# haidog-yaqub/EzAudio

Hardware: AMD Instinct MI355X
Metric: denoising steps/sec (EzAudio-XL, 10 s latent, CFG on) (higher is better)
Workload: dtype bf16

## Files before the change

ezaudio_amd/csrc/attn.hip:

```cpp
#include "common.h"

namespace {

typedef __attribute__((ext_vector_type(4))) short s16x4;

__device__ __forceinline__ float pair_max(float x) {
    const auto r = __builtin_amdgcn_permlane32_swap(__float_as_uint(x), __float_as_uint(x), false, false);
    return fmaxf(__uint_as_float(r[0]), __uint_as_float(r[1]));
}
__device__ __forceinline__ float pair_sum(float x) {
    const auto r = __builtin_amdgcn_permlane32_swap(__float_as_uint(x), __float_as_uint(x), false, false);
    return __uint_as_float(r[0]) + __uint_as_float(r[1]);
}

template <int DH>
struct HeadGeom;
template <>
struct HeadGeom<64> { static constexpr int DQK = 64, DV = 64; };
template <>
struct HeadGeom<72> { static constexpr int DQK = 80, DV = 96; };

template <int DH, int NKH, bool ZQ = false, int QT = 64>
__global__ __launch_bounds__(128 * NKH) void k_attn(AttnArgs a) {
    static_assert(QT == 64 || (QT == 32 && NKH == 4), "32-query tiles: the 8-wave fused-projection form only");
    constexpr int NQS = QT / 32;
    constexpr int NT = 128 * NKH;
    constexpr int TK = 32 * NKH;
    constexpr int DQK = HeadGeom<DH>::DQK;
    constexpr int DV = HeadGeom<DH>::DV;
    constexpr int NKS = DQK / 16;
    constexpr int NDT = DV / 32;
    constexpr int KSTR = DQK * 2 + 16;
    constexpr int VSTR = 192;
    static_assert(DV * 2 <= VSTR, "V row");
    constexpr int KBYTES = TK * KSTR, VBYTES = TK * VSTR;
    constexpr int BUF = KBYTES + VBYTES;
    constexpr int KCH = TK * DQK * 2 / 16;
    constexpr int VCPR = DV / 8;
    constexpr int VCH = TK * VCPR;
    constexpr int KPT = (KCH + NT - 1) / NT, VPT = (VCH + NT - 1) / NT;
    static_assert(KPT <= 3 && VPT <= 3, "staging registers");
    constexpr int DN = DV >= 96 ? 96 : 64;
    constexpr int DW = DQK;
    constexpr int DS = DQK;
    constexpr int NRS = QT == 64 ? 3 : 4;
    constexpr int PSTAGE = (QT + DN) * 128, PRING = 2 * NRS * PSTAGE;
    constexpr int PRED = 4 * 64 * DS * 4, PQS = QT * DQK * 2;
    constexpr int SMEM = NKH == 4 ? (2 * BUF > PRED + PQS ? (2 * BUF > PRING ? 2 * BUF : PRING) : (PRED + PQS > PRING ? PRED + PQS : PRING)) : 2 * BUF;
    constexpr int ZX = ZQ ? QT * 8 + 2 * DQK * 4 : 0;
    __shared__ __attribute__((aligned(16))) char smem[SMEM + ZX];

    int Lq_ = a.Lq;
    asm("" : "+s"(Lq_) : "s"(a.q), "s"(a.k), "s"(a.v), "s"(a.kmask), "s"(a.out), "s"(a.ldo), "s"(a.B), "s"(a.H), "s"(a.Lk), "s"(a.Lqp), "s"(a.Lkp), "s"(a.xu), "s"(a.ldu),
        "s"(a.xw), "s"(a.ldw), "s"(a.xw_rows), "s"(a.xK), "s"(a.xcd_map), "s"(a.nq), "s"(a.ppx), "s"(a.mnq), "s"(a.mH), "s"(a.q_raw), "s"(a.ts), "s"(a.xk2), "s"(a.zstat_in),
        "s"(a.zs_stride), "s"(a.zparts), "s"(a.klen));
    const int tid = threadIdx.x;
    const int lane = tid & 63;
    const int wave = tid >> 6;
    const int qs = QT == 64 ? (wave & 1) : 0, kh = QT == 64 ? (wave >> 1) : (wave & 3);
    const bool active = QT == 64 || __builtin_amdgcn_readfirstlane(wave) < 4;
    const int r32 = lane & 31, hi = lane >> 5;
    int qt, h, b;
    if (a.xcd_map) {
        const int xcd = blockIdx.x & 7, sl = blockIdx.x >> 3;
        const int sq = ez_div(sl, a.mnq);
        const int pair = xcd * a.ppx + sq;
        qt = sl - sq * a.nq;
        if (pair >= a.B * a.H) return;
        b = ez_div(pair, a.mH); h = pair - b * a.H;
    } else {
        qt = blockIdx.x; h = blockIdx.y; b = blockIdx.z;
    }
    const int q0 = qt * QT + qs * 32;
    const long bh = (long)b * a.H + h;
    int Lk = a.Lk;
    if constexpr (!ZQ) {
        if (a.klen) {
            Lk = __builtin_amdgcn_readfirstlane(a.klen[b]);
            if (qt * QT >= Lk) {
                for (int i = tid; i < QT * (DH / 4); i += NT) {
                    const int r = i / (DH / 4), g = i - r * (DH / 4);
                    if (qt * QT + r < a.Lq)
                        *reinterpret_cast<uint2*>(a.out + ((long)b * a.Lq + qt * QT + r) * a.ldo + h * DH + 4 * g) = make_uint2(0u, 0u);
                }
                return;
            }
        }
    }
    unsigned long long* ts = (a.ts && tid < 64) ? a.ts + 8 * (long)blockIdx.x : nullptr;
    if (ts && lane == 0) { ts[0] = __builtin_readcyclecounter(); ts[6] = ez_stamp_start(); }

    const bf16_t* Q = a.q + (bh * a.Lqp + q0 + r32) * DQK + 8 * hi;
    const char* Kg = reinterpret_cast<const char*>(a.k + bh * a.Lkp * DQK);
    const bf16_t* Vg = a.v + bh * DV * (long)a.Lkp;
    const uint8_t* km = a.kmask ? a.kmask + (long)b * a.Lk : nullptr;

    bf16x8 qf[NKS];
    if (NKH == 4 && a.xu) {
        if constexpr (NKH == 4) {
            constexpr int FN = DN / 32;
            constexpr int NPART = QT == 64 ? 4 : 8;
            const int rowb = b * a.Lq;
            float2* zrow_l = reinterpret_cast<float2*>(smem + SMEM);
            float* zgc_l = reinterpret_cast<float*>(smem + SMEM + QT * 8);
            ZStatRegs zst;
            float4 zgc_reg = make_float4(0.f, 0.f, 0.f, 0.f);
            const int wave_u = __builtin_amdgcn_readfirstlane(wave);
            const char* gA = reinterpret_cast<const char*>(a.xu);
            const char* gW = reinterpret_cast<const char*>(a.xw);
            const int nt = a.xK / 64;
            auto z_request = [&]() {
                if constexpr (ZQ) {
                    if (tid < 4 * QT) {
                        int qr = qt * QT + (tid >> 2);
                        qr = qr < a.Lq ? qr : a.Lq - 1;
                        z_row_stats_load(a.zstat_in + (rowb + qr), a.zs_stride, a.zparts, tid & 3, zst);
                    }
                    if (tid < 2 * (DH / 4)) {
                        const int which = tid >= DH / 4, t4 = tid - which * (DH / 4);
                        zgc_reg = *reinterpret_cast<const float4*>((which ? a.zC : a.zG) + h * DH + 4 * t4);
                    }
                }
            };
            f32x16 acc[FN];
#pragma unroll
            for (int j = 0; j < FN; ++j)
#pragma unroll
                for (int r = 0; r < 16; ++r) acc[j][r] = 0.f;
            if constexpr (QT == 32) {
                constexpr int NCH = (32 + DW) * 8, NW1 = (NCH - NT) / 64;
                static_assert(NCH > NT && NCH <= 2 * NT && (NCH - NT) % 64 == 0, "two passes, whole waves");
                uint32_t off0, off1;
                {
                    const int row = tid >> 3, c = tid & 7;
                    if (row < 32) {
                        int grow = rowb + qt * 32 + row;
                        grow = grow < rowb + a.Lq - 1 ? grow : rowb + a.Lq - 1;
                        off0 = (uint32_t)(grow * a.ldu + ((c ^ ((row >> 1) & 7)) << 3)) * 2u;
                    } else {
                        const int r2 = row - 32;
                        int gr = h * DH + r2;
                        gr = gr < a.xw_rows - 1 ? gr : a.xw_rows - 1;
                        off0 = (uint32_t)(gr * a.ldw + ((c ^ ((r2 >> 1) & 7)) << 3)) * 2u;
                    }
                    const int r2 = (tid >> 3) + 32;
                    int gr = h * DH + r2;
                    gr = gr < a.xw_rows - 1 ? gr : a.xw_rows - 1;
                    off1 = (uint32_t)(gr * a.ldw + ((c ^ ((r2 >> 1) & 7)) << 3)) * 2u;
                }
                const char* g0 = wave_u < 4 ? gA : gW;
                const bool two = wave_u < NW1;
                auto stage2 = [&](int sidx) {
                    char* dst = smem + (sidx % NRS) * 2 * PSTAGE + wave_u * 1024;
#pragma unroll
                    for (int sub = 0; sub < 2; ++sub) {
                        const long ko = (long)(2 * sidx + sub) * 128;
                        __builtin_amdgcn_global_load_lds((const __attribute__((address_space(1))) void*)(g0 + ko + off0),
                                                         (__attribute__((address_space(3))) void*)(dst + sub * PSTAGE), 16, 0, 0);
                        if (two)
                            __builtin_amdgcn_global_load_lds((const __attribute__((address_space(1))) void*)(gW + ko + off1),
                                                             (__attribute__((address_space(3))) void*)(dst + sub * PSTAGE + NT * 16), 16, 0, 0);
                    }
                };
                const int ns = nt >> 1;
                stage2(0);
                z_request();
                if (ns > 1) stage2(1);
                if (ns > 2) stage2(2);
                const int sub = wave_u >> 2, kq = wave_u & 3;
                const uint32_t fo = r32 * 128 + (((2 * kq + hi) ^ ((r32 >> 1) & 7)) << 4);
                for (int sidx = 0; sidx < ns; ++sidx) {
                    const int younger = ns - 1 - sidx < NRS - 2 ? ns - 1 - sidx : NRS - 2;
                    if (two) {
                        if (younger >= 2) asm volatile("s_waitcnt vmcnt(8)" ::: "memory");
                        else if (younger == 1) asm volatile("s_waitcnt vmcnt(4)" ::: "memory");
                        else asm volatile("s_waitcnt vmcnt(0)" ::: "memory");
                    } else {
                        if (younger >= 2) asm volatile("s_waitcnt vmcnt(4)" ::: "memory");
                        else if (younger == 1) asm volatile("s_waitcnt vmcnt(2)" ::: "memory");
                        else asm volatile("s_waitcnt vmcnt(0)" ::: "memory");
                    }
                    __builtin_amdgcn_s_barrier();
                    if (sidx + NRS - 1 < ns) stage2(sidx + NRS - 1);
                    const char* cT = smem + (sidx % NRS) * 2 * PSTAGE + sub * PSTAGE;
                    const bf16x8 af = *reinterpret_cast<const bf16x8*>(cT + fo);
#pragma unroll
                    for (int j = 0; j < FN; ++j) {
                        const bf16x8 bfr = *reinterpret_cast<const bf16x8*>(cT + 32 * 128 + fo + j * 4096);
                        acc[j] = __builtin_amdgcn_mfma_f32_32x32x16_bf16(bfr, af, acc[j], 0, 0, 0);
                    }
#pragma unroll
                    for (int j = 0; j < FN; ++j) asm volatile("" : "+a"(acc[j]));
                }
            } else {
            const int mh = wave & 1, kq = wave >> 1;
            uint32_t aoff[1], boff[(DW * 8 + NT - 1) / NT];
            stage_offsets<64, NT>(aoff, a.ldu, rowb + qt * 64, rowb + a.Lq - 1, tid);
            stage_offsets<DW, NT>(boff, a.ldw, h * DH, a.xw_rows - 1, tid);
            auto stage = [&](int t) {
                char* dst = smem + (t % 3) * PSTAGE + wave_u * 1024;
                stage_tile<64, NT>(gA + (long)t * 128, aoff, dst, tid);
                stage_tile<DW, NT>(gW + (long)t * 128, boff, dst + 64 * 128, tid);
            };
            const bool two = (DW * 8 > NT) && (wave_u * 64 + NT < DW * 8);
            stage(0);
            if (nt > 1) stage(1);
            z_request();
            const uint32_t fo = r32 * 128 + (((2 * kq + hi) ^ ((r32 >> 1) & 7)) << 4);
            if (a.xk2 && (nt & 1) == 0) {
                const int ns = nt >> 1;
                auto stage2 = [&](int sidx) {
                    char* dst = smem + (sidx % 3) * 2 * PSTAGE + wave_u * 1024;
#pragma unroll
                    for (int sub = 0; sub < 2; ++sub) {
                        stage_tile<64, NT>(gA + (long)(2 * sidx + sub) * 128, aoff, dst + sub * PSTAGE, tid);
                        stage_tile<DW, NT>(gW + (long)(2 * sidx + sub) * 128, boff, dst + sub * PSTAGE + 64 * 128, tid);
                    }
                };
                if (ns > 1) stage2(1);
                for (int sidx = 0; sidx < ns; ++sidx) {
                    if (sidx + 1 < ns) {
                        if (two) asm volatile("s_waitcnt vmcnt(6)" ::: "memory"); else asm volatile("s_waitcnt vmcnt(4)" ::: "memory");
                    } else {
                        asm volatile("s_waitcnt vmcnt(0)" ::: "memory");
                    }
                    __builtin_amdgcn_s_barrier();
                    if (sidx + 2 < ns) stage2(sidx + 2);
#pragma unroll
                    for (int sub = 0; sub < 2; ++sub) {
                        const char* cT = smem + (sidx % 3) * 2 * PSTAGE + sub * PSTAGE;
                        const bf16x8 af = *reinterpret_cast<const bf16x8*>(cT + fo + mh * 4096);
#pragma unroll
                        for (int j = 0; j < FN; ++j) {
                            const bf16x8 bfr = *reinterpret_cast<const bf16x8*>(cT + 64 * 128 + fo + j * 4096);
                            acc[j] = __builtin_amdgcn_mfma_f32_32x32x16_bf16(bfr, af, acc[j], 0, 0, 0);
                        }
                    }
#pragma unroll
                    for (int j = 0; j < FN; ++j) asm volatile("" : "+a"(acc[j]));
                }
            } else
            for (int t = 0; t < nt; ++t) {
                if (t + 1 < nt) {
                    if (two) asm volatile("s_waitcnt vmcnt(3)" ::: "memory"); else asm volatile("s_waitcnt vmcnt(2)" ::: "memory");
                } else {
                    asm volatile("s_waitcnt vmcnt(0)" ::: "memory");
                }
                __builtin_amdgcn_s_barrier();
                if (t + 2 < nt) stage(t + 2);
                const char* cT = smem + (t % 3) * PSTAGE;
                const bf16x8 af = *reinterpret_cast<const bf16x8*>(cT + fo + mh * 4096);
#pragma unroll
                for (int j = 0; j < FN; ++j) {
                    const bf16x8 bfr = *reinterpret_cast<const bf16x8*>(cT + 64 * 128 + fo + j * 4096);
                    acc[j] = __builtin_amdgcn_mfma_f32_32x32x16_bf16(bfr, af, acc[j], 0, 0, 0);
                }
#pragma unroll
                for (int j = 0; j < FN; ++j) asm volatile("" : "+a"(acc[j]));
            }
            }
#pragma unroll
            for (int j = 0; j < FN; ++j) asm volatile("s_nop 7\n\ts_nop 7\n\ts_nop 3" : "+a"(acc[j]));
            if constexpr (ZQ) {
                if (tid < 4 * QT) {
                    const float2 mr = z_row_stats_finish(zst, a.zparts, tid & 3, a.zD, a.zeps);
                    if ((tid & 3) == 0) zrow_l[tid >> 2] = mr;
                }
                if (tid < 2 * (DH / 4)) {
                    const int which = tid >= DH / 4, t4 = tid - which * (DH / 4);
                    *reinterpret_cast<float4*>(zgc_l + which * DQK + 4 * t4) = zgc_reg;
                }
            }
            __syncthreads();
            float* red = reinterpret_cast<float*>(smem);
            {
                const int pw = QT == 64 ? (wave >> 1) : wave, prow = QT == 64 ? 32 * (wave & 1) + r32 : r32;
#pragma unroll
                for (int j = 0; j < FN; ++j)
#pragma unroll
                    for (int g = 0; g < 4; ++g) {
                        const int col = 32 * j + 8 * g + 4 * hi;
                        if (col < DS)
                            *reinterpret_cast<float4*>(red + ((pw * QT + prow) * DS + col)) =
                                make_float4(acc[j][4 * g], acc[j][4 * g + 1], acc[j][4 * g + 2], acc[j][4 * g + 3]);
                    }
            }
            __syncthreads();
            if (QT == 64 || tid < 8 * QT) {
                constexpr int CP = DH / 8;
                bf16_t* qs_l = reinterpret_cast<bf16_t*>(smem + PRED);
                const int row = tid >> 3, part = tid & 7;
                float v[CP];
                float s1 = 0.f;
                const float2 zmr = ZQ ? zrow_l[row] : make_float2(0.f, 1.f);
                const float zmu = zmr.x, zr = zmr.y;
#pragma unroll
                for (int e = 0; e < CP; ++e) {
                    const int col = part * CP + e;
                    if constexpr (QT == 64) {
                        v[e] = red[(0 * 64 + row) * DS + col] + red[(1 * 64 + row) * DS + col] + red[(2 * 64 + row) * DS + col] +
                               red[(3 * 64 + row) * DS + col];
                    } else {
                        float t = red[row * DS + col];
#pragma unroll
                        for (int w = 1; w < NPART; ++w) t += red[(w * QT + row) * DS + col];
                        v[e] = t;
                    }
                    if constexpr (ZQ) v[e] = fmaf(zr, v[e], fmaf(-zr * zmu, zgc_l[col], zgc_l[DQK + col]));
                    s1 += v[e];
                }
                s1 = oct_sum(s1);
                const float mean = s1 * (1.f / DH);
                float s2 = 0.f;
#pragma unroll
                for (int e = 0; e < CP; ++e) { const float d = v[e] - mean; s2 += d * d; }
                s2 = oct_sum(s2);
                const float rstd = rsqrtf(s2 * (1.f / DH) + 1e-5f);
#pragma unroll
                for (int e = 0; e < CP; ++e) {
                    const int col = part * CP + e;
                    qs_l[row * DQK + col] = f2bf((v[e] - mean) * rstd * a.qn_w[col] + a.qn_b[col]);
                }
                if (DQK > DH && part == 0)
                    for (int col = DH; col < DQK; ++col) qs_l[row * DQK + col] = 0;
            }
            __syncthreads();
            {
                const bf16_t* qs_l = reinterpret_cast<const bf16_t*>(smem + PRED);
#pragma unroll
                for (int ks = 0; ks < NKS; ++ks) qf[ks] = *reinterpret_cast<const bf16x8*>(qs_l + (32 * qs + r32) * DQK + 16 * ks + 8 * hi);
            }
            __syncthreads();
        }
    } else if (a.q_raw) {
        int qr = q0 + r32;
        if (qr >= a.Lq) qr = a.Lq - 1;
        const float* src = a.q_raw + ((long)b * a.Lq + qr) * a.ld_qraw + h * DH + 8 * hi;
        float v[NKS][8];
        float s = 0.f;
#pragma unroll
        for (int ks = 0; ks < NKS; ++ks) {
            const bool ok = 16 * ks + 8 * hi < DH;
            const float4 lo = ok ? *reinterpret_cast<const float4*>(src + 16 * ks) : make_float4(0.f, 0.f, 0.f, 0.f);
            const float4 hh = ok ? *reinterpret_cast<const float4*>(src + 16 * ks + 4) : make_float4(0.f, 0.f, 0.f, 0.f);
            v[ks][0] = lo.x; v[ks][1] = lo.y; v[ks][2] = lo.z; v[ks][3] = lo.w;
            v[ks][4] = hh.x; v[ks][5] = hh.y; v[ks][6] = hh.z; v[ks][7] = hh.w;
#pragma unroll
            for (int e = 0; e < 8; ++e) s += v[ks][e];
        }
        s += __shfl_xor(s, 32, 64);
        const float mean = s * (1.f / DH);
        float q2 = 0.f;
#pragma unroll
        for (int ks = 0; ks < NKS; ++ks)
            if (16 * ks + 8 * hi < DH) {
#pragma unroll
                for (int e = 0; e < 8; ++e) { const float d = v[ks][e] - mean; q2 += d * d; }
            }
        q2 += __shfl_xor(q2, 32, 64);
        const float rstd = rsqrtf(q2 * (1.f / DH) + 1e-5f);
#pragma unroll
        for (int ks = 0; ks < NKS; ++ks) {
            const int d0 = 16 * ks + 8 * hi;
            const bool ok = d0 < DH;
            const int dw = ok ? d0 : 0;
            union { bf16x8 v; uint32_t u[4]; } pk;
#pragma unroll
            for (int e = 0; e < 4; ++e) {
                const float y0 = ok ? (v[ks][2 * e] - mean) * rstd * a.qn_w[dw + 2 * e] + a.qn_b[dw + 2 * e] : 0.f;
                const float y1 = ok ? (v[ks][2 * e + 1] - mean) * rstd * a.qn_w[dw + 2 * e + 1] + a.qn_b[dw + 2 * e + 1] : 0.f;
                pk.u[e] = pack_bf2(y0, y1);
            }
            qf[ks] = pk.v;
        }
    } else {
#pragma unroll
        for (int ks = 0; ks < NKS; ++ks) qf[ks] = *reinterpret_cast<const bf16x8*>(Q + 16 * ks);
    }

    uint4 k0 = {}, k1 = {}, k2 = {}, v0 = {}, v1 = {}, v2 = {};
    uint32_t koff[3], voff[3];
#pragma unroll
    for (int i = 0; i < 3; ++i) {
        int ck = tid + NT * i, cv = tid + NT * i;
        ck = ck < KCH ? ck : KCH - 1;
        cv = cv < VCH ? cv : VCH - 1;
        koff[i] = (uint32_t)ck * 16u;
        voff[i] = (uint32_t)cv * 16u;
    }
    const __amdgpu_buffer_rsrc_t krs = __builtin_amdgcn_make_buffer_rsrc(const_cast<char*>(Kg), 0, a.Lkp * DQK * 2, 0x00020000);
    const __amdgpu_buffer_rsrc_t vrs = __builtin_amdgcn_make_buffer_rsrc(const_cast<bf16_t*>(Vg), 0, DV * a.Lkp * 2, 0x00020000);
    auto kchunk = [&](int i, int key0) -> uint4 {
        return __builtin_bit_cast(uint4, __builtin_amdgcn_raw_buffer_load_b128(krs, (int)koff[i], key0 * DQK * 2, 0));
    };
    auto vchunk = [&](int i, int key0) -> uint4 {
        return __builtin_bit_cast(uint4, __builtin_amdgcn_raw_buffer_load_b128(vrs, (int)voff[i], key0 * DV * 2, 0));
    };
    auto kstore = [&](int i, char* kb, const uint4& val) {
        const int c = tid + NT * i;
        if (c < KCH) *reinterpret_cast<uint4*>(kb + (c / (DQK / 8)) * KSTR + (c % (DQK / 8)) * 16) = val;
    };
    auto vstore = [&](int i, char* vb, const uint4& val) {
        const int c = tid + NT * i;
        if (c < VCH) *reinterpret_cast<uint4*>(vb + (c / VCPR) * VSTR + (c % VCPR) * 16) = val;
    };
#define LOAD_TILE(t)                                   \
    do {                                               \
        const int key0_ = (t) * TK;                    \
        k0 = kchunk(0, key0_);                         \
        k1 = kchunk(1, key0_);                         \
        if constexpr (KPT > 2) k2 = kchunk(2, key0_);  \
        v0 = vchunk(0, key0_);                         \
        v1 = vchunk(1, key0_);                         \
        if constexpr (VPT > 2) v2 = vchunk(2, key0_);  \
    } while (0)
#define WRITE_TILE(buf)                                \
    do {                                               \
        char* kb_ = smem + (buf) * BUF;                \
        char* vb_ = kb_ + KBYTES;                      \
        kstore(0, kb_, k0);                            \
        kstore(1, kb_, k1);                            \
        if constexpr (KPT > 2) kstore(2, kb_, k2);     \
        vstore(0, vb_, v0);                            \
        vstore(1, vb_, v1);                            \
        if constexpr (VPT > 2) vstore(2, vb_, v2);     \
    } while (0)

    f32x16 o[NDT];
#pragma unroll
    for (int t = 0; t < NDT; ++t)
#pragma unroll
        for (int r = 0; r < 16; ++r) o[t][r] = 0.f;
    float m = -1e30f, lsum = 0.f;
    constexpr float RESCALE_THR = 4.0f;
    const float c = 1.4426950408889634f * rsqrtf((float)DH);

    if (NKH == 4 && __builtin_amdgcn_readfirstlane(threadIdx.x) >= 256) __builtin_amdgcn_s_setprio(1);
    const int ntiles = (Lk + TK - 1) / TK;
    LOAD_TILE(0);
    WRITE_TILE(0);
    __syncthreads();
    if (ts && lane == 0) ts[1] = __builtin_readcyclecounter();
    for (int t = 0; t < ntiles; ++t) {
        if (t + 1 < ntiles) LOAD_TILE(t + 1);
        const char* kb = smem + (t & 1) * BUF;
        const char* vb = kb + KBYTES;
        const char* vtr = vb + (32 * kh + 4 * hi + ((lane & 15) >> 2)) * VSTR + ((lane & 16) + 4 * (lane & 3)) * 2;
        const int key0 = t * TK + kh * 32;
        if (active && key0 < Lk) {
            const int kidx = key0 + r32;
            bool kv = kidx < Lk;
            if (km) kv = kv && (km[kidx < Lk ? kidx : 0] != 0);
            const uint32_t ball = (uint32_t)__ballot(kv);
            const uint32_t tmask = ball >> (4 * hi);
            const bool full = ball == 0xffffffffu;
            f32x16 s;
            {
                const bf16x8 kf0 = *reinterpret_cast<const bf16x8*>(kb + (kh * 32 + r32) * KSTR + hi * 16);
                asm("s_nop 1\n\tv_mfma_f32_32x32x16_bf16 %0, %1, %2, 0" : "=&v"(s) : "v"(kf0), "v"(qf[0]));
            }
#pragma unroll
            for (int ks = 1; ks < NKS; ++ks) {
                const bf16x8 kf = *reinterpret_cast<const bf16x8*>(kb + (kh * 32 + r32) * KSTR + (2 * ks + hi) * 16);
                if (ks + 1 < NKS) asm("s_nop 1\n\tv_mfma_f32_32x32x16_bf16 %0, %1, %2, %0" : "+v"(s) : "v"(kf), "v"(qf[ks]));
                else asm("s_nop 1\n\tv_mfma_f32_32x32x16_bf16 %0, %1, %2, %0\n\ts_nop 7\n\ts_nop 7\n\ts_nop 3" : "+v"(s) : "v"(kf), "v"(qf[ks]));
            }
            float tmax = -1e30f;
            if (full) {
#pragma unroll
                for (int r = 0; r < 16; ++r) tmax = fmaxf(tmax, s[r]);
                tmax *= c;
            } else {
#pragma unroll
                for (int r = 0; r < 16; ++r) {
                    const bool v = (tmask >> ((r & 3) + 8 * (r >> 2))) & 1u;
                    s[r] = v ? s[r] * c : -1e30f;
                    tmax = fmaxf(tmax, s[r]);
                }
            }
            tmax = pair_max(tmax);
            if (!__all(tmax <= m + RESCALE_THR)) {
                const float mnew = fmaxf(m, tmax);
                const float alpha = __builtin_amdgcn_exp2f(m - mnew);
                m = mnew;
                lsum *= alpha;
#pragma unroll
                for (int tt = 0; tt < NDT; ++tt)
#pragma unroll
                    for (int r = 0; r < 16; ++r) o[tt][r] *= alpha;
            }
            float psum = 0.f;
            float p[16];
            if (full) {
                const f32x2 c2 = {c, c}, nm2 = {-m, -m};
                f32x2 ps2 = {0.f, 0.f};
#pragma unroll
                for (int r = 0; r < 16; r += 2) {
                    f32x2 x = {s[r], s[r + 1]};
                    x = __builtin_elementwise_fma(x, c2, nm2);
                    p[r] = __builtin_amdgcn_exp2f(x[0]);
                    p[r + 1] = __builtin_amdgcn_exp2f(x[1]);
                    const f32x2 pp = {p[r], p[r + 1]};
                    ps2 += pp;
                }
                psum = ps2[0] + ps2[1];
            } else {
#pragma unroll
                for (int r = 0; r < 16; ++r) {
                    const bool v = (tmask >> ((r & 3) + 8 * (r >> 2))) & 1u;
                    p[r] = v ? __builtin_amdgcn_exp2f(s[r] - m) : 0.f;
                    psum += p[r];
                }
            }
            psum = pair_sum(psum);
            lsum += psum;
#pragma unroll
            for (int step = 0; step < 2; ++step) {
                union { bf16x8 v; uint32_t u[4]; } pf;
#pragma unroll
                for (int e = 0; e < 4; ++e) pf.u[e] = pack_bf2(p[8 * step + 2 * e], p[8 * step + 2 * e + 1]);
#pragma unroll
                for (int tt = 0; tt < NDT; ++tt) {
                    const char* vp = vtr + (16 * step) * VSTR + 64 * tt;
                    union { bf16x8 v; s16x4 h2[2]; } vf;
                    vf.h2[0] = __builtin_amdgcn_ds_read_tr16_b64_v4i16((__attribute__((address_space(3))) s16x4*)(vp));
                    vf.h2[1] = __builtin_amdgcn_ds_read_tr16_b64_v4i16((__attribute__((address_space(3))) s16x4*)(vp + 8 * VSTR));
                    asm("s_nop 1\n\tv_mfma_f32_32x32x16_bf16 %0, %1, %2, %0" : "+v"(o[tt]) : "v"(vf.v), "v"(pf.v));
                }
            }
        }
        if (t + 1 < ntiles) WRITE_TILE((t + 1) & 1);
        __syncthreads();
    }

    if (ts && lane == 0) ts[2] = __builtin_readcyclecounter();
#pragma unroll
    for (int tt = 0; tt < NDT; ++tt) asm volatile("s_nop 7\n\ts_nop 7\n\ts_nop 3" : "+v"(o[tt]));
    constexpr int NG = DH / 8;
    constexpr int NW = 2 * NKH;
    float4* xo = reinterpret_cast<float4*>(smem);
    float* xml = reinterpret_cast<float*>(smem + NKH * NQS * NG * 64 * 16);
    static_assert(SMEM >= NKH * NQS * NG * 64 * 16 + NKH * NQS * 2 * 32 * 4, "exchange area must fit the staging buffers");
    if (active) {
#pragma unroll
        for (int G = 0; G < NG; ++G)
            xo[((kh * NQS + qs) * NG + G) * 64 + lane] = make_float4(o[G / 4][4 * (G % 4)], o[G / 4][4 * (G % 4) + 1], o[G / 4][4 * (G % 4) + 2], o[G / 4][4 * (G % 4) + 3]);
        if (hi == 0) {
            xml[((kh * NQS + qs) * 2 + 0) * 32 + r32] = m;
            xml[((kh * NQS + qs) * 2 + 1) * 32 + r32] = lsum;
        }
    }
    __syncthreads();
    if (ts && lane == 0) ts[4] = __builtin_readcyclecounter();
    float wgt[NKH];
    {
        float mk[NKH], mm = -1e30f;
#pragma unroll
        for (int k = 0; k < NKH; ++k) { mk[k] = xml[((k * NQS + qs) * 2 + 0) * 32 + r32]; mm = fmaxf(mm, mk[k]); }
        float l = 0.f;
#pragma unroll
        for (int k = 0; k < NKH; ++k) { wgt[k] = __builtin_amdgcn_exp2f(mk[k] - mm); l = fmaf(xml[((k * NQS + qs) * 2 + 1) * 32 + r32], wgt[k], l); }
        const float inv = 1.f / l;
#pragma unroll
        for (int k = 0; k < NKH; ++k) wgt[k] *= inv;
    }
    const int qrow = q0 + r32;
    bf16_t* orow = a.out + ((long)b * a.Lq + (qrow < a.Lq ? qrow : a.Lq - 1)) * a.ldo + h * DH + 4 * hi;
#pragma unroll
    for (int i = 0; i < (NQS * NG + NW - 1) / NW; ++i) {
        const int G = (wave + i * NW) / NQS;
        if (G < NG) {
            float4 acc = make_float4(0.f, 0.f, 0.f, 0.f);
#pragma unroll
            for (int k = 0; k < NKH; ++k) {
                const float4 v = xo[((k * NQS + qs) * NG + G) * 64 + lane];
                acc.x = fmaf(v.x, wgt[k], acc.x); acc.y = fmaf(v.y, wgt[k], acc.y); acc.z = fmaf(v.z, wgt[k], acc.z); acc.w = fmaf(v.w, wgt[k], acc.w);
            }
            if (qrow < a.Lq) {
                uint2 v;
                v.x = pack_bf2(acc.x, acc.y);
                v.y = pack_bf2(acc.z, acc.w);
                if constexpr (!ZQ) {
                    if (a.klen && qrow >= Lk) v = make_uint2(0u, 0u);
                }
                if (a.wt) st8_wt(orow + 8 * G, v); else *reinterpret_cast<uint2*>(orow + 8 * G) = v;
            }
        }
    }
    if (ts && lane == 0) { asm volatile("s_waitcnt vmcnt(0)" ::: "memory"); ts[3] = __builtin_readcyclecounter(); ts[7] = __builtin_amdgcn_s_memrealtime(); }
}

#undef LOAD_TILE
#undef WRITE_TILE

}

int launch_attention(const AttnArgs& a0, hipStream_t st) {
    AttnArgs a = a0;
    if (a.b0 > 0) {
        const int DQK = a.dh == 64 ? 64 : 80, DV = a.dh == 64 ? 64 : 96;
        const long b0 = a.b0;
        if (a.q) a.q += b0 * a.H * a.Lqp * DQK;
        if (a.k) a.k += b0 * a.H * a.Lkp * DQK;
        if (a.v) a.v += b0 * a.H * DV * (long)a.Lkp;
        if (a.kmask) a.kmask += b0 * a.Lk;
        if (a.out) a.out += b0 * a.Lq * a.ldo;
        if (a.q_raw) a.q_raw += b0 * a.Lq * a.ld_qraw;
        if (a.xu) a.xu += b0 * a.Lq * a.ldu;
        if (a.zstat_in) a.zstat_in += b0 * a.Lq;
        if (a.klen) a.klen += b0;
        a.b0 = 0;
    }
    const long nwg64 = (long)((a.Lq + 63) / 64) * a.H * a.B;
    int nkh = a.nkh;
    if (nkh != 2 && nkh != 4) nkh = nwg64 <= 512 ? 4 : 2;
    if (a.Lkp % 128) nkh = 2;
    if (a.xu && nkh != 4) return 1;
    if (a.dh != 64 && a.dh != 72) return 1;
    if (a.klen && (a.xu || a.q_raw || a.Lq != a.Lk)) return 1;
    const bool zq = a.xu && a.zstat_in;
    if (zq && !(a.zG && a.zC && a.zparts > 0 && a.zparts <= Z_MAXP && a.zs_stride > 0 && a.zw > 0)) return 1;
    const bool q32 = zq && nkh == 4 && (a.xK / 64) % 2 == 0 && a.xcd_map && (a.qtile == 32 || (a.qtile == 0 && nwg64 <= 128));
    const int QT = q32 ? 32 : 64;
    a.nq = (a.Lq + QT - 1) / QT;
    a.ppx = (a.B * a.H + 7) / 8;
    a.mnq = ez_magic(a.nq); a.mH = ez_magic(a.H);
    dim3 grid(a.nq, a.H, a.B);
    if (a.xcd_map) grid = dim3(8 * a.ppx * a.nq, 1, 1);
    if (a.ts && (long)grid.x * grid.y * grid.z > a.ts_cap) a.ts = nullptr;
    if (q32) {
        if (a.dh == 64) hipLaunchKernelGGL((k_attn<64, 4, true, 32>), grid, dim3(512), 0, st, a);
        else hipLaunchKernelGGL((k_attn<72, 4, true, 32>), grid, dim3(512), 0, st, a);
        return 0;
    }
    if (a.dh == 64) {
        if (nkh == 4 && zq) hipLaunchKernelGGL((k_attn<64, 4, true>), grid, dim3(512), 0, st, a);
        else if (nkh == 4) hipLaunchKernelGGL((k_attn<64, 4>), grid, dim3(512), 0, st, a);
        else hipLaunchKernelGGL((k_attn<64, 2>), grid, dim3(256), 0, st, a);
    } else {
        if (nkh == 4 && zq) hipLaunchKernelGGL((k_attn<72, 4, true>), grid, dim3(512), 0, st, a);
        else if (nkh == 4) hipLaunchKernelGGL((k_attn<72, 4>), grid, dim3(512), 0, st, a);
        else hipLaunchKernelGGL((k_attn<72, 2>), grid, dim3(256), 0, st, a);
    }
    return 0;
}
```

Before: 272.9.

## Give each wave a private K-slice in the fused Q-projection of 32-query attention

```diff
diff --git a/ezaudio_amd/csrc/attn.hip b/ezaudio_amd/csrc/attn.hip
--- a/ezaudio_amd/csrc/attn.hip
+++ b/ezaudio_amd/csrc/attn.hip
@@ -43,10 +43,18 @@
     constexpr int DN = DV >= 96 ? 96 : 64;
     constexpr int DW = DQK;
     constexpr int DS = DQK;
-    constexpr int NRS = QT == 64 ? 3 : 4;
-    constexpr int PSTAGE = (QT + DN) * 128, PRING = 2 * NRS * PSTAGE;
+    constexpr int NRS = 3;
+    constexpr int PSTAGE = (64 + DN) * 128;
     constexpr int PRED = 4 * 64 * DS * 4, PQS = QT * DQK * 2;
-    constexpr int SMEM = NKH == 4 ? (2 * BUF > PRED + PQS ? (2 * BUF > PRING ? 2 * BUF : PRING) : (PRED + PQS > PRING ? PRED + PQS : PRING)) : 2 * BUF;
+    constexpr int PR = 32 + DW;
+    constexpr int NIP = PR * 4 / 64, NIS = (PR * 2 + 63) / 64;
+    static_assert(PR * 4 % 64 == 0, "a pair of k-steps is whole DMA instructions");
+    constexpr int PAIRB = PR * 64, SINGB = NIS * 1024, WSLOT = 2 * PAIRB + SINGB;
+    constexpr int DSP = DS + 8;
+    static_assert(QT != 32 || (32 * DSP * 4 + PQS <= WSLOT && PAIRB + (32 + DN) * 64 <= WSLOT && (32 + DN) * 32 <= SINGB), "partials, Qs and the dropped W rows stay inside a wave's slots");
+    constexpr int PRING = QT == 32 ? 8 * WSLOT : 2 * NRS * PSTAGE;
+    constexpr int PREDQ = QT == 32 ? 0 : PRED + PQS;
+    constexpr int SMEM = NKH == 4 ? (2 * BUF > PREDQ ? (2 * BUF > PRING ? 2 * BUF : PRING) : (PREDQ > PRING ? PREDQ : PRING)) : 2 * BUF;
     constexpr int ZX = ZQ ? QT * 8 + 2 * DQK * 4 : 0;
     __shared__ __attribute__((aligned(16))) char smem[SMEM + ZX];
 
@@ -100,6 +108,7 @@
         if constexpr (NKH == 4) {
             constexpr int FN = DN / 32;
             constexpr int NPART = QT == 64 ? 4 : 8;
+            constexpr int QOFF = QT == 64 ? PRED : 32 * DSP * 4;
             const int rowb = b * a.Lq;
             float2* zrow_l = reinterpret_cast<float2*>(smem + SMEM);
             float* zgc_l = reinterpret_cast<float*>(smem + SMEM + QT * 8);
@@ -128,67 +137,95 @@
 #pragma unroll
                 for (int r = 0; r < 16; ++r) acc[j][r] = 0.f;
             if constexpr (QT == 32) {
-                constexpr int NCH = (32 + DW) * 8, NW1 = (NCH - NT) / 64;
-                static_assert(NCH > NT && NCH <= 2 * NT && (NCH - NT) % 64 == 0, "two passes, whole waves");
-                uint32_t off0, off1;
+                uint32_t poff[NIP], soff[NIS];
                 {
-                    const int row = tid >> 3, c = tid & 7;
-                    if (row < 32) {
-                        int grow = rowb + qt * 32 + row;
-                        grow = grow < rowb + a.Lq - 1 ? grow : rowb + a.Lq - 1;
-                        off0 = (uint32_t)(grow * a.ldu + ((c ^ ((row >> 1) & 7)) << 3)) * 2u;
-                    } else {
-                        const int r2 = row - 32;
-                        int gr = h * DH + r2;
-                        gr = gr < a.xw_rows - 1 ? gr : a.xw_rows - 1;
-                        off0 = (uint32_t)(gr * a.ldw + ((c ^ ((r2 >> 1) & 7)) << 3)) * 2u;
-                    }
-                    const int r2 = (tid >> 3) + 32;
-                    int gr = h * DH + r2;
-                    gr = gr < a.xw_rows - 1 ? gr : a.xw_rows - 1;
-                    off1 = (uint32_t)(gr * a.ldw + ((c ^ ((r2 >> 1) & 7)) << 3)) * 2u;
-                }
-                const char* g0 = wave_u < 4 ? gA : gW;
-                const bool two = wave_u < NW1;
-                auto stage2 = [&](int sidx) {
-                    char* dst = smem + (sidx % NRS) * 2 * PSTAGE + wave_u * 1024;
-#pragma unroll
-                    for (int sub = 0; sub < 2; ++sub) {
-                        const long ko = (long)(2 * sidx + sub) * 128;
-                        __builtin_amdgcn_global_load_lds((const __attribute__((address_space(1))) void*)(g0 + ko + off0),
-                                                         (__attribute__((address_space(3))) void*)(dst + sub * PSTAGE), 16, 0, 0);
-                        if (two)
-                            __builtin_amdgcn_global_load_lds((const __attribute__((address_space(1))) void*)(gW + ko + off1),
-                                                             (__attribute__((address_space(3))) void*)(dst + sub * PSTAGE + NT * 16), 16, 0, 0);
-                    }
+                    const int xlast = rowb + a.Lq - 1, wlast = a.xw_rows - 1;
+#pragma unroll
+                    for (int n = 0; n < NIP; ++n) {
+                        const int i = 64 * n + lane, R = i >> 2, c = (i & 3) ^ ((R >> 2) & 3);
+                        int gr = n < 2 ? rowb + qt * 32 + R : h * DH + R - 32;
+                        const int last = n < 2 ? xlast : wlast;
+                        gr = gr < last ? gr : last;
+                        poff[n] = (uint32_t)(gr * (n < 2 ? a.ldu : a.ldw) + (c << 3)) * 2u;
+                    }
+#pragma unroll
+                    for (int n = 0; n < NIS; ++n) {
+                        int i = 64 * n + lane;
+                        i = i < PR * 2 ? i : PR * 2 - 1;
+                        const int R = i >> 1, c = (i & 1) ^ ((R >> 3) & 1);
+                        int gr = n < 1 ? rowb + qt * 32 + R : h * DH + R - 32;
+                        const int last = n < 1 ? xlast : wlast;
+                        gr = gr < last ? gr : last;
+                        soff[n] = (uint32_t)(gr * (n < 1 ? a.ldu : a.ldw) + (c << 3)) * 2u;
+                    }
+                }
+                const int nks = a.xK >> 4, kbase = nks >> 3, krem = nks & 7;
+                const int nk = kbase + (wave_u < krem ? 1 : 0);
+                const int ks0 = wave_u * kbase + (wave_u < krem ? wave_u : krem);
+                const int np = nk >> 1;
+                const bool sg = nk & 1;
+                char* wslot = smem + wave_u * WSLOT;
+                const char* gAk = gA + (long)ks0 * 32;
+                const char* gWk = gW + (long)ks0 * 32;
+                auto pair_req = [&](int p) {
+                    char* dst = wslot + (p & 1) * PAIRB;
+#pragma unroll
+                    for (int n = 0; n < NIP; ++n)
+                        __builtin_amdgcn_global_load_lds((const __attribute__((address_space(1))) void*)((n < 2 ? gAk : gWk) + (long)p * 64 + poff[n]),
+                                                         (__attribute__((address_space(3))) void*)(dst + n * 1024), 16, 0, 0);
                 };
-                const int ns = nt >> 1;
-                stage2(0);
+                auto single_req = [&]() {
+                    char* dst = wslot + 2 * PAIRB;
+#pragma unroll
+                    for (int n = 0; n < NIS; ++n)
+                        __builtin_amdgcn_global_load_lds((const __attribute__((address_space(1))) void*)((n < 1 ? gAk : gWk) + (long)np * 64 + soff[n]),
+                                                         (__attribute__((address_space(3))) void*)(dst + n * 1024), 16, 0, 0);
+                };
+                if (np > 0) pair_req(0); else if (sg) single_req();
                 z_request();
-                if (ns > 1) stage2(1);
-                if (ns > 2) stage2(2);
-                const int sub = wave_u >> 2, kq = wave_u & 3;
-                const uint32_t fo = r32 * 128 + (((2 * kq + hi) ^ ((r32 >> 1) & 7)) << 4);
-                for (int sidx = 0; sidx < ns; ++sidx) {
-                    const int younger = ns - 1 - sidx < NRS - 2 ? ns - 1 - sidx : NRS - 2;
-                    if (two) {
-                        if (younger >= 2) asm volatile("s_waitcnt vmcnt(8)" ::: "memory");
-                        else if (younger == 1) asm volatile("s_waitcnt vmcnt(4)" ::: "memory");
-                        else asm volatile("s_waitcnt vmcnt(0)" ::: "memory");
-                    } else {
-                        if (younger >= 2) asm volatile("s_waitcnt vmcnt(4)" ::: "memory");
-                        else if (younger == 1) asm volatile("s_waitcnt vmcnt(2)" ::: "memory");
-                        else asm volatile("s_waitcnt vmcnt(0)" ::: "memory");
-                    }
-                    __builtin_amdgcn_s_barrier();
-                    if (sidx + NRS - 1 < ns) stage2(sidx + NRS - 1);
-                    const char* cT = smem + (sidx % NRS) * 2 * PSTAGE + sub * PSTAGE;
-                    const bf16x8 af = *reinterpret_cast<const bf16x8*>(cT + fo);
+                if (np > 1) pair_req(1);
+                if (np > 0 && sg) single_req();
+                const uint32_t sw2 = (r32 >> 2) & 3;
+                const uint32_t fop0 = r32 * 64 + ((hi ^ sw2) << 4), fop1 = r32 * 64 + (((2 + hi) ^ sw2) << 4);
+                const uint32_t fos = r32 * 32 + ((hi ^ ((r32 >> 3) & 1)) << 4);
+                auto single_mma = [&]() {
+                    const char* cT = wslot + 2 * PAIRB;
+                    const bf16x8 af = *reinterpret_cast<const bf16x8*>(cT + fos);
 #pragma unroll
                     for (int j = 0; j < FN; ++j) {
-                        const bf16x8 bfr = *reinterpret_cast<const bf16x8*>(cT + 32 * 128 + fo + j * 4096);
+                        const bf16x8 bfr = *reinterpret_cast<const bf16x8*>(cT + (32 + 32 * j) * 32 + fos);
                         acc[j] = __builtin_amdgcn_mfma_f32_32x32x16_bf16(bfr, af, acc[j], 0, 0, 0);
                     }
+                };
+                if (np == 0 && sg) {
+                    asm volatile("s_waitcnt vmcnt(0)" ::: "memory");
+                    single_mma();
+                }
+                for (int p = 0; p < np; ++p) {
+                    const bool nxt = p + 1 < np;
+                    if (nxt && sg && p == 0) asm volatile("s_waitcnt vmcnt(%0)" :: "n"(NIP + NIS) : "memory");
+                    else if (nxt) asm volatile("s_waitcnt vmcnt(%0)" :: "n"(NIP) : "memory");
+                    else asm volatile("s_waitcnt vmcnt(0)" ::: "memory");
+                    const char* cT = wslot + (p & 1) * PAIRB;
+                    bf16x8 af[2], bfr[2][FN];
+                    af[0] = *reinterpret_cast<const bf16x8*>(cT + fop0);
+                    af[1] = *reinterpret_cast<const bf16x8*>(cT + fop1);
+#pragma unroll
+                    for (int j = 0; j < FN; ++j) {
+                        bfr[0][j] = *reinterpret_cast<const bf16x8*>(cT + (32 + 32 * j) * 64 + fop0);
+                        bfr[1][j] = *reinterpret_cast<const bf16x8*>(cT + (32 + 32 * j) * 64 + fop1);
+                    }
+                    if (p + 2 < np) {
+#pragma unroll
+                        for (int j = 0; j < FN; ++j) asm volatile("" : "+v"(bfr[0][j]), "+v"(bfr[1][j]));
+                        asm volatile("s_waitcnt lgkmcnt(0)" : "+v"(af[0]), "+v"(af[1]) :: "memory");
+                        pair_req(p + 2);
+                    }
+#pragma unroll
+                    for (int s = 0; s < 2; ++s)
+#pragma unroll
+                        for (int j = 0; j < FN; ++j) acc[j] = __builtin_amdgcn_mfma_f32_32x32x16_bf16(bfr[s][j], af[s], acc[j], 0, 0, 0);
+                    if (sg && p == (np > 1 ? 1 : 0)) single_mma();
 #pragma unroll
                     for (int j = 0; j < FN; ++j) asm volatile("" : "+a"(acc[j]));
                 }
@@ -271,7 +308,9 @@
                     *reinterpret_cast<float4*>(zgc_l + which * DQK + 4 * t4) = zgc_reg;
                 }
             }
-            __syncthreads();
+            if constexpr (QT == 64) __syncthreads();
+            constexpr int RP = QT == 64 ? DS : DSP;
+            constexpr int RW = QT == 64 ? 64 * DS : WSLOT / 4;
             float* red = reinterpret_cast<float*>(smem);
             {
                 const int pw = QT == 64 ? (wave >> 1) : wave, prow = QT == 64 ? 32 * (wave & 1) + r32 : r32;
@@ -281,14 +320,14 @@
                     for (int g = 0; g < 4; ++g) {
                         const int col = 32 * j + 8 * g + 4 * hi;
                         if (col < DS)
-                            *reinterpret_cast<float4*>(red + ((pw * QT + prow) * DS + col)) =
+                            *reinterpret_cast<float4*>(red + (pw * RW + prow * RP + col)) =
                                 make_float4(acc[j][4 * g], acc[j][4 * g + 1], acc[j][4 * g + 2], acc[j][4 * g + 3]);
                     }
             }
             __syncthreads();
             if (QT == 64 || tid < 8 * QT) {
                 constexpr int CP = DH / 8;
-                bf16_t* qs_l = reinterpret_cast<bf16_t*>(smem + PRED);
+                bf16_t* qs_l = reinterpret_cast<bf16_t*>(smem + QOFF);
                 const int row = tid >> 3, part = tid & 7;
                 float v[CP];
                 float s1 = 0.f;
@@ -296,14 +335,14 @@
                 const float zmu = zmr.x, zr = zmr.y;
 #pragma unroll
                 for (int e = 0; e < CP; ++e) {
-                    const int col = part * CP + e;
+                    const int col = QT == 64 ? part * CP + e : part + 8 * e;
                     if constexpr (QT == 64) {
                         v[e] = red[(0 * 64 + row) * DS + col] + red[(1 * 64 + row) * DS + col] + red[(2 * 64 + row) * DS + col] +
                                red[(3 * 64 + row) * DS + col];
                     } else {
-                        float t = red[row * DS + col];
-#pragma unroll
-                        for (int w = 1; w < NPART; ++w) t += red[(w * QT + row) * DS + col];
+                        float t = red[row * RP + col];
+#pragma unroll
+                        for (int w = 1; w < NPART; ++w) t += red[w * RW + row * RP + col];
                         v[e] = t;
                     }
                     if constexpr (ZQ) v[e] = fmaf(zr, v[e], fmaf(-zr * zmu, zgc_l[col], zgc_l[DQK + col]));
@@ -318,7 +357,7 @@
                 const float rstd = rsqrtf(s2 * (1.f / DH) + 1e-5f);
 #pragma unroll
                 for (int e = 0; e < CP; ++e) {
-                    const int col = part * CP + e;
+                    const int col = QT == 64 ? part * CP + e : part + 8 * e;
                     qs_l[row * DQK + col] = f2bf((v[e] - mean) * rstd * a.qn_w[col] + a.qn_b[col]);
                 }
                 if (DQK > DH && part == 0)
@@ -326,7 +365,7 @@
             }
             __syncthreads();
             {
-                const bf16_t* qs_l = reinterpret_cast<const bf16_t*>(smem + PRED);
+                const bf16_t* qs_l = reinterpret_cast<const bf16_t*>(smem + QOFF);
 #pragma unroll
                 for (int ks = 0; ks < NKS; ++ks) qf[ks] = *reinterpret_cast<const bf16x8*>(qs_l + (32 * qs + r32) * DQK + 16 * ks + 8 * hi);
             }
@@ -620,7 +659,7 @@
     if (a.klen && (a.xu || a.q_raw || a.Lq != a.Lk)) return 1;
     const bool zq = a.xu && a.zstat_in;
     if (zq && !(a.zG && a.zC && a.zparts > 0 && a.zparts <= Z_MAXP && a.zs_stride > 0 && a.zw > 0)) return 1;
-    const bool q32 = zq && nkh == 4 && (a.xK / 64) % 2 == 0 && a.xcd_map && (a.qtile == 32 || (a.qtile == 0 && nwg64 <= 128));
+    const bool q32 = zq && nkh == 4 && a.xK >= 128 && a.xK % 16 == 0 && a.ldu % 8 == 0 && a.ldw % 8 == 0 && a.xcd_map && (a.qtile == 32 || (a.qtile == 0 && nwg64 <= 128));
     const int QT = q32 ? 32 : 64;
     a.nq = (a.Lq + QT - 1) / QT;
     a.ppx = (a.B * a.H + 7) / 8;
```

Result: slower. 269.5 (-1.2%).
